# constantinpape/torch-em

Measured on AMD Instinct MI355X. Metric: voxels/sec fwd+bwd, UNet3d 1x128^3 bs=2, higher is better.
Workload: dtype f32-class (forward convs on normalised activations: fp32 operands split into 2 fp16 terms = 22 mantissa bits, lo plane scaled by 2^12 with its own fp32 accumulator, 3 fp16 MFMAs per product; other forward convs 3 bf16 terms / 6 MFMAs; data-gradient convs 2 bf16 terms / 3 MFMAs (16-bit products); WEI

## Files before the change

### torch_em_amd/csrc/conv1x1_stream.hip

```cpp
#include "tem_common.h"
#include "tem_act.h"
#include "conv_split.h"
#include "conv_internal.h"
#include "conv_arith.h"

template <int NS, bool F16, int CT, typename T>
__global__ __launch_bounds__(256) void k_conv1x1_stream(const T* __restrict__ x, int64_t x_ld,
                                                        const unsigned short* __restrict__ wp,
                                                        const float* __restrict__ bias, T* __restrict__ y,
                                                        int64_t y_ld, const T* __restrict__ ref, int64_t ref_ld,
                                                        int64_t NV, int Cin, int Cout, int act, int64_t nmt,
                                                        unsigned* __restrict__ amax) {
    const int lane = threadIdx.x & 63, wv = threadIdx.x >> 6;
    float amx = 0.f;
    const int r = lane & 31, kh = lane >> 5;
    const int ctg = blockIdx.y;
    const int nks = Cin >> 4;
    const uint4* wfrag = reinterpret_cast<const uint4*>(wp) + lane;
    for (int64_t mt = (int64_t)blockIdx.x * 4 + wv; mt < nmt; mt += (int64_t)gridDim.x * 4) {
        const int64_t v = mt * 32 + r;
        const bool vok = v < NV;
        const T* xr = x + (vok ? v : 0) * x_ld + kh * 8;
        floatx16 acc[CT];
#pragma unroll
        for (int ct = 0; ct < CT; ++ct)
#pragma unroll
            for (int k = 0; k < 16; ++k) acc[ct][k] = 0.f;
        for (int ks = 0; ks < nks; ++ks) {
            uint4 t[NS];
            if constexpr (sizeof(T) == 2) {
                static_assert(sizeof(T) == 4 || NS == 1, "16-bit storage: one-term modes only");
                t[0] = make_uint4(0u, 0u, 0u, 0u);
                if (vok) t[0] = *reinterpret_cast<const uint4*>(xr + ks * 16);
            } else {
                float4 a0 = make_float4(0.f, 0.f, 0.f, 0.f), a1 = a0;
                if (vok) {
                    a0 = act_ld4(xr + ks * 16);
                    a1 = act_ld4(xr + ks * 16 + 4);
                }
                float rem[8] = {a0.x, a0.y, a0.z, a0.w, a1.x, a1.y, a1.z, a1.w};
#pragma unroll
                for (int p = 0; p < NS; ++p) {
                    unsigned wds[4];
#pragma unroll
                    for (int e = 0; e < 4; ++e) {
                        const unsigned h = pk16<F16>(rem[2 * e], rem[2 * e + 1]);
                        wds[e] = h;
                        if (p + 1 < NS) {
                            rem[2 * e] -= lo16<F16>(h);
                            rem[2 * e + 1] -= hi16<F16>(h);
                        }
                    }
                    t[p] = make_uint4(wds[0], wds[1], wds[2], wds[3]);
                }
            }
#pragma unroll
            for (int ct = 0; ct < CT; ++ct) {
                const int nt = ctg * CT + ct;
                if (nt * 32 < Cout) {
                    const uint4* f = wfrag + ((int64_t)(nt * nks + ks) * NS) * 64;
                    uint4 b[NS];
#pragma unroll
                    for (int p = 0; p < NS; ++p) b[p] = f[p * 64];
#pragma unroll
                    for (int o = NS - 1; o >= 0; --o)
#pragma unroll
                        for (int i = 0; i <= o; ++i) acc[ct] = mfma16<F16>(b[o - i], t[i], acc[ct]);
                }
            }
        }
        if (vok) {
#pragma unroll
            for (int ct = 0; ct < CT; ++ct) {
#pragma unroll
                for (int q4 = 0; q4 < 4; ++q4) {
                    const int co = (ctg * CT + ct) * 32 + 8 * q4 + 4 * kh;
                    if (co < Cout) {
                        float4 o = make_float4(acc[ct][4 * q4], acc[ct][4 * q4 + 1], acc[ct][4 * q4 + 2], acc[ct][4 * q4 + 3]);
                        if (bias) {
                            const float4 b4 = *reinterpret_cast<const float4*>(bias + co);
                            o.x += b4.x;
                            o.y += b4.y;
                            o.z += b4.z;
                            o.w += b4.w;
                        }
                        o.x = act_apply_b(o.x, act);
                        o.y = act_apply_b(o.y, act);
                        o.z = act_apply_b(o.z, act);
                        o.w = act_apply_b(o.w, act);
                        if (ref) {
                            const float4 rv = act_ld4(ref + v * ref_ld + co);
                            o.x = rv.x > 0.f ? o.x : 0.f;
                            o.y = rv.y > 0.f ? o.y : 0.f;
                            o.z = rv.z > 0.f ? o.z : 0.f;
                            o.w = rv.w > 0.f ? o.w : 0.f;
                        }
                        act_st4(y + v * y_ld + co, o);
                        amx = tem_amax4(amx, o.x, o.y, o.z, o.w);
                    }
                }
            }
        }
    }
    if (amax) tem_amax_commit(amax, amx);
}

template <int NS, bool F16, typename T>
static void stream_launch(const TemConvCall& c, const T* x, int64_t x_ld, const float* wp, const float* bias, T* y, int64_t y_ld,
                          const T* ref, int64_t ref_ld, int64_t NV, int Cin, int Cout, int act, hipStream_t s) {
    const int64_t nmt = (NV + 31) / 32;
    const int ntile = Cout / 32;
    const int CT = ntile >= 2 ? 2 : 1;
    const int ngroups = (ntile + CT - 1) / CT;
    int64_t gx = (nmt + 3) / 4;
    if (gx > 8192) gx = 8192;
    const dim3 grid((unsigned)gx, (unsigned)ngroups);
    unsigned* const amax = c.take_output_amax();
    if (CT == 2)
        hipLaunchKernelGGL((k_conv1x1_stream<NS, F16, 2, T>), grid, dim3(256), 0, s, x, x_ld, (const unsigned short*)wp, bias, y, y_ld,
                           ref, ref_ld, NV, Cin, Cout, act, nmt, amax);
    else
        hipLaunchKernelGGL((k_conv1x1_stream<NS, F16, 1, T>), grid, dim3(256), 0, s, x, x_ld, (const unsigned short*)wp, bias, y, y_ld,
                           ref, ref_ld, NV, Cin, Cout, act, nmt, amax);
}

void tem_conv1x1_stream(const TemConvCall& c, const float* x, int64_t x_ld, const float* wp, const float* bias, float* y, int64_t y_ld,
                        const float* ref, int64_t ref_ld, const TemConvShape& sh, int act, int mode, hipStream_t s) {
    const int st = c.stx, Cin = sh.Cin, Cout = sh.Cout;
    const int64_t NV = sh.NV();
    auto go = [&](auto ns, auto f16, auto t) {
        using T = decltype(t);
        stream_launch<ns(), f16(), T>(c, (const T*)x, x_ld, wp, bias, (T*)y, y_ld, (const T*)ref, ref_ld, NV, Cin, Cout, act, s);
    };
    const TemArith& a = tem_arith(mode);
    if (st == TEM_ST_F16) go(TemInt<1>{}, TemBool<true>{}, tem_f16{});
    else if (st == TEM_ST_BF16) go(TemInt<1>{}, TemBool<false>{}, tem_bf16{});
    else if (a.planes == 3) go(TemInt<3>{}, TemBool<false>{}, float{});
    else if (a.planes == 2) go(TemInt<2>{}, TemBool<false>{}, float{});
    else tem_select_bool(a.elem == TEM_EL_F16, [&](auto f16) { go(TemInt<1>{}, f16, float{}); });
}
```

### torch_em_amd/csrc/capi.hip

```cpp
#include "tem_common.h"
#include "conv_internal.h"
#include "tem_act.h"
#include <stdarg.h>
#include <string.h>

static thread_local char g_err[512] = "";

void tem_set_error(const char* fmt, ...) {
    va_list ap;
    va_start(ap, fmt);
    vsnprintf(g_err, sizeof(g_err), fmt, ap);
    va_end(ap);
}

extern "C" const char* tem_last_error(void) { return g_err; }

struct TemOption {
    const char* name;
    long long def;
};
static const TemOption g_opt_table[TEM_OPT_COUNT] = {
    {"wgrad_zs", 3},
    {"wgrad_zs_persist", 1},
    {"wgrad_sums", 1},
    {"wgrad_sums_min_mb", 128},
    {"fwd_persistent", -1},
    {"conv_fwd_variant", -1},
    {"conv1x1_stream", 1},
    {"fwd_ksplit_chunks", 0},
    {"wgrad_cus", 256},
    {"upsample_generic", 0},
    {"team_min_units", 0},
    {"zr_splitk", 1},
    {"zr_wide", 1},
    {"zr_tile_blocks", 1},
    {"dice_vox", 1},
    {"upsample2_ch8", 1},
    {"pool_vec8", 2},
    {"fp32_zr", 1},
    {"zr_pair", 1},
};
static long long g_opt_val[TEM_OPT_COUNT];
static bool g_opt_set[TEM_OPT_COUNT];

long long tem_option(int id) {
    if (id < 0 || id >= TEM_OPT_COUNT) return 0;
    return __atomic_load_n(&g_opt_set[id], __ATOMIC_RELAXED) ? __atomic_load_n(&g_opt_val[id], __ATOMIC_RELAXED)
                                                            : g_opt_table[id].def;
}
static int opt_find(const char* name) {
    if (!name) return -1;
    for (int i = 0; i < TEM_OPT_COUNT; ++i)
        if (!strcmp(name, g_opt_table[i].name)) return i;
    return -1;
}
extern "C" int tem_set_option(const char* name, int64_t value) {
    const int id = opt_find(name);
    TEM_REQUIRE(id >= 0, "tem_set_option: unknown option '%s'", name ? name : "(null)");
    __atomic_store_n(&g_opt_val[id], (long long)value, __ATOMIC_RELAXED);
    __atomic_store_n(&g_opt_set[id], true, __ATOMIC_RELAXED);
    return TEM_OK;
}
extern "C" int tem_get_option(const char* name, int64_t* value) {
    const int id = opt_find(name);
    TEM_REQUIRE(id >= 0 && value, "tem_get_option: unknown option '%s'", name ? name : "(null)");
    *value = (int64_t)tem_option(id);
    return TEM_OK;
}
extern "C" int tem_version(void) { return 100; }

extern "C" int tem_device_cus(void) {
    int dev = 0;
    if (hipGetDevice(&dev) != hipSuccess) return TEM_ELAUNCH;
    hipDeviceProp_t prop;
    if (hipGetDeviceProperties(&prop, dev) != hipSuccess) return TEM_ELAUNCH;
    return prop.multiProcessorCount;
}
int tem_ncu() {
    static int ncu = 0;
    if (!ncu) {
        ncu = tem_device_cus();
        if (ncu <= 0) ncu = 256;
    }
    return ncu;
}

#define TT_V 64
#define TT_C 32

__global__ __launch_bounds__(256) void k_nchw_to_nhwc(const float* __restrict__ src, float* __restrict__ dst,
                                                      int64_t dst_ld, int C, int64_t V, int64_t vtiles, int ctiles) {
    __shared__ float tile[TT_C][TT_V + 1];
    int64_t ntiles = vtiles * ctiles;
    int n = blockIdx.y;
    for (int64_t t = blockIdx.x; t < ntiles; t += gridDim.x) {
        int ct = (int)(t % ctiles);
        int64_t vt = t / ctiles;
        int64_t v0 = vt * TT_V;
        int c0 = ct * TT_C;
        for (int i = threadIdx.x; i < TT_C * TT_V; i += 256) {
            int c = i / TT_V, v = i % TT_V;
            float val = 0.f;
            if (c0 + c < C && v0 + v < V) val = src[((int64_t)n * C + c0 + c) * V + v0 + v];
            tile[c][v] = val;
        }
        __syncthreads();
        for (int i = threadIdx.x; i < TT_C * TT_V; i += 256) {
            int v = i / TT_C, c = i % TT_C;
            if (c0 + c < C && v0 + v < V) dst[((int64_t)n * V + v0 + v) * dst_ld + c0 + c] = tile[c][v];
        }
        __syncthreads();
    }
}

__global__ __launch_bounds__(256) void k_nhwc_to_nchw(const float* __restrict__ src, int64_t src_ld,
                                                      float* __restrict__ dst, int C, int64_t V, int64_t vtiles,
                                                      int ctiles) {
    __shared__ float tile[TT_C][TT_V + 1];
    int64_t ntiles = vtiles * ctiles;
    int n = blockIdx.y;
    for (int64_t t = blockIdx.x; t < ntiles; t += gridDim.x) {
        int ct = (int)(t % ctiles);
        int64_t vt = t / ctiles;
        int64_t v0 = vt * TT_V;
        int c0 = ct * TT_C;
        for (int i = threadIdx.x; i < TT_C * TT_V; i += 256) {
            int v = i / TT_C, c = i % TT_C;
            float val = 0.f;
            if (c0 + c < C && v0 + v < V) val = src[((int64_t)n * V + v0 + v) * src_ld + c0 + c];
            tile[c][v] = val;
        }
        __syncthreads();
        for (int i = threadIdx.x; i < TT_C * TT_V; i += 256) {
            int c = i / TT_V, v = i % TT_V;
            if (c0 + c < C && v0 + v < V) dst[((int64_t)n * C + c0 + c) * V + v0 + v] = tile[c][v];
        }
        __syncthreads();
    }
}

extern "C" int tem_nchw_to_nhwc(const float* src, float* dst, int64_t dst_ld, int N, int C, int64_t V,
                                tem_stream_t stream) {
    TEM_REQUIRE(src && dst && N > 0 && C > 0 && V > 0 && dst_ld >= C, "tem_nchw_to_nhwc: bad arguments");
    int64_t vtiles = tem_cdiv(V, TT_V);
    int ctiles = (int)tem_cdiv(C, TT_C);
    int64_t nt = vtiles * ctiles;
    dim3 grid((unsigned)(nt > 4096 ? 4096 : nt), N);
    hipLaunchKernelGGL(k_nchw_to_nhwc, grid, dim3(256), 0, (hipStream_t)stream, src, dst, dst_ld, C, V, vtiles, ctiles);
    TEM_CHECK_LAUNCH("tem_nchw_to_nhwc");
    return TEM_OK;
}

extern "C" int tem_nhwc_to_nchw(const float* src, int64_t src_ld, float* dst, int N, int C, int64_t V,
                                tem_stream_t stream) {
    TEM_REQUIRE(src && dst && N > 0 && C > 0 && V > 0 && src_ld >= C, "tem_nhwc_to_nchw: bad arguments");
    int64_t vtiles = tem_cdiv(V, TT_V);
    int ctiles = (int)tem_cdiv(C, TT_C);
    int64_t nt = vtiles * ctiles;
    dim3 grid((unsigned)(nt > 4096 ? 4096 : nt), N);
    hipLaunchKernelGGL(k_nhwc_to_nchw, grid, dim3(256), 0, (hipStream_t)stream, src, src_ld, dst, C, V, vtiles, ctiles);
    TEM_CHECK_LAUNCH("tem_nhwc_to_nchw");
    return TEM_OK;
}

#define STD_BLOCKS 256

__global__ __launch_bounds__(256) void k_std_partial(const float* __restrict__ x, int64_t L, double* __restrict__ part) {
    int n = blockIdx.y;
    const float* row = x + (int64_t)n * L;
    double s = 0.0, ss = 0.0;
    for (int64_t i = (int64_t)blockIdx.x * 256 + threadIdx.x; i < L; i += (int64_t)gridDim.x * 256) {
        double v = (double)row[i];
        s += v;
        ss += v * v;
    }
    s = tem_wave_sum_d(s);
    ss = tem_wave_sum_d(ss);
    __shared__ double sh[2][4];
    int w = threadIdx.x >> 6;
    if ((threadIdx.x & 63) == 0) { sh[0][w] = s; sh[1][w] = ss; }
    __syncthreads();
    if (threadIdx.x == 0) {
        part[((int64_t)n * gridDim.x + blockIdx.x) * 2 + 0] = sh[0][0] + sh[0][1] + sh[0][2] + sh[0][3];
        part[((int64_t)n * gridDim.x + blockIdx.x) * 2 + 1] = sh[1][0] + sh[1][1] + sh[1][2] + sh[1][3];
    }
}

__global__ __launch_bounds__(256) void k_std_apply(const float* __restrict__ x, float* __restrict__ y, int64_t L,
                                                   const double* __restrict__ part, int nblk, float eps) {
    int n = blockIdx.y;
    __shared__ float sh_mean, sh_inv;
    if (threadIdx.x == 0) {
        double s = 0.0, ss = 0.0;
        for (int b = 0; b < nblk; ++b) {
            s += part[((int64_t)n * nblk + b) * 2 + 0];
            ss += part[((int64_t)n * nblk + b) * 2 + 1];
        }
        double mean = s / (double)L;
        double var = ss / (double)L - mean * mean;
        if (var < 0.0) var = 0.0;
        sh_mean = (float)mean;
        sh_inv = (float)(1.0 / (sqrt(var) + (double)eps));
    }
    __syncthreads();
    float mean = sh_mean, inv = sh_inv;
    const float* row = x + (int64_t)n * L;
    float* out = y + (int64_t)n * L;
    for (int64_t i = (int64_t)blockIdx.x * 256 + threadIdx.x; i < L; i += (int64_t)gridDim.x * 256)
        out[i] = (row[i] - mean) * inv;
}

extern "C" int tem_standardize(const float* x, float* y, int N, int64_t L, float eps, void* ws, int64_t ws_bytes,
                               tem_stream_t stream) {
    TEM_REQUIRE(x && y && ws && N > 0 && L > 0, "tem_standardize: bad arguments");
    int nblk = (int)(tem_cdiv(L, 256) < STD_BLOCKS ? tem_cdiv(L, 256) : STD_BLOCKS);
    if ((int64_t)N * nblk * 2 * (int64_t)sizeof(double) > ws_bytes) {
        tem_set_error("tem_standardize: workspace too small (%lld bytes needed)",
                      (long long)((int64_t)N * nblk * 2 * sizeof(double)));
        return TEM_EWS;
    }
    hipLaunchKernelGGL(k_std_partial, dim3(nblk, N), dim3(256), 0, (hipStream_t)stream, x, L, (double*)ws);
    hipLaunchKernelGGL(k_std_apply, dim3(nblk, N), dim3(256), 0, (hipStream_t)stream, x, y, L, (const double*)ws, nblk, eps);
    TEM_CHECK_LAUNCH("tem_standardize");
    return TEM_OK;
}

__global__ __launch_bounds__(256) void k_act_bwd(const float* __restrict__ gy, const float* __restrict__ y,
                                                 float* __restrict__ gx, int64_t n, int act) {
    for (int64_t i = (int64_t)blockIdx.x * 256 + threadIdx.x; i < n; i += (int64_t)gridDim.x * 256) {
        float yv = y[i], g = gy[i];
        gx[i] = (act == TEM_ACT_SIGMOID) ? g * yv * (1.f - yv) : ((yv > 0.f) ? g : 0.f);
    }
}

extern "C" int tem_act_bwd(const float* gy, const float* y, float* gx, int64_t n, int act, tem_stream_t stream) {
    TEM_REQUIRE(gy && y && gx && n > 0, "tem_act_bwd: bad arguments");
    TEM_REQUIRE(act == TEM_ACT_RELU || act == TEM_ACT_SIGMOID, "tem_act_bwd: Invalid activation: %d", act);
    hipLaunchKernelGGL(k_act_bwd, dim3(tem_grid_1d(n, 256)), dim3(256), 0, (hipStream_t)stream, gy, y, gx, n, act);
    TEM_CHECK_LAUNCH("tem_act_bwd");
    return TEM_OK;
}
```

### torch_em_amd/csrc/tem_common.h

```cpp
#pragma once
#include <hip/hip_runtime.h>
#include <stdint.h>
#include <stdio.h>
#include "../../include/tem_hip.h"

void tem_set_error(const char* fmt, ...);

enum {
    TEM_OPT_WGRAD_ZS = 0,
    TEM_OPT_WGRAD_ZS_PERSIST,
    TEM_OPT_WGRAD_SUMS,
    TEM_OPT_WGRAD_SUMS_MIN_MB,
    TEM_OPT_FWD_PERSISTENT,
    TEM_OPT_CONV_FWD_VARIANT,
    TEM_OPT_CONV1X1_STREAM,
    TEM_OPT_FWD_KSPLIT_CHUNKS,
    TEM_OPT_WGRAD_CUS,
    TEM_OPT_UPSAMPLE_GENERIC,
    TEM_OPT_TEAM_MIN_UNITS,
    TEM_OPT_ZR_SPLITK,
    TEM_OPT_ZR_WIDE,
    TEM_OPT_ZR_TILE_BLOCKS,
    TEM_OPT_DICE_VOX,
    TEM_OPT_UPSAMPLE2_CH8,
    TEM_OPT_POOL_VEC8,
    TEM_OPT_FP32_ZR,
    TEM_OPT_ZR_PAIR,
    TEM_OPT_COUNT
};
long long tem_option(int id);
int tem_ncu();

#define TEM_REQUIRE(cond, ...)                 \
    do {                                       \
        if (!(cond)) {                         \
            tem_set_error(__VA_ARGS__);        \
            return TEM_EINVAL;                 \
        }                                      \
    } while (0)

#define TEM_TRY(call)                          \
    do {                                       \
        const int rc__ = (call);               \
        if (rc__ != TEM_OK) return rc__;       \
    } while (0)

#define TEM_CHECK_LAUNCH(name)                                                   \
    do {                                                                         \
        hipError_t e__ = hipGetLastError();                                      \
        if (e__ != hipSuccess) {                                                 \
            tem_set_error("%s: launch failed: %s", name, hipGetErrorString(e__)); \
            return TEM_ELAUNCH;                                                  \
        }                                                                        \
    } while (0)

static inline int64_t tem_cdiv(int64_t a, int64_t b) { return (a + b - 1) / b; }
static inline int64_t tem_align_up(int64_t a, int64_t b) { return tem_cdiv(a, b) * b; }

static inline int tem_grid_1d(int64_t work_items, int block, int max_blocks = 256 * 8) {
    int64_t g = tem_cdiv(work_items, block);
    if (g > max_blocks) g = max_blocks;
    if (g < 1) g = 1;
    return (int)g;
}

#define TEM_WAVE 64

__device__ __forceinline__ float tem_amax4(float m, float a, float b, float c, float d) {
    return __builtin_fmaxf(__builtin_fmaxf(m, __builtin_fmaxf(__builtin_fabsf(a), __builtin_fabsf(b))),
                           __builtin_fmaxf(__builtin_fabsf(c), __builtin_fabsf(d)));
}
__device__ __forceinline__ void tem_amax_commit(unsigned* amax, float m) {
    unsigned u = __builtin_bit_cast(unsigned, m);
#pragma unroll
    for (int o = 32; o > 0; o >>= 1) u = max(u, (unsigned)__shfl_xor((int)u, o, 64));
    if ((threadIdx.x & 63) == 0 && u > __atomic_load_n(amax, __ATOMIC_RELAXED)) atomicMax(amax, u);
}

__device__ __forceinline__ float tem_wave_sum(float v) {
#pragma unroll
    for (int o = 32; o > 0; o >>= 1) v += __shfl_xor(v, o, 64);
    return v;
}
__device__ __forceinline__ double tem_wave_sum_d(double v) {
#pragma unroll
    for (int o = 32; o > 0; o >>= 1) v += __shfl_xor(v, o, 64);
    return v;
}

__device__ __forceinline__ int tem_xcd_remap(int bid, int nwg) {
    const int nx = 8;
    int q = nwg / nx, r = nwg % nx;
    int xcd = bid % nx, idx = bid / nx;
    int base = (xcd < r) ? xcd * (q + 1) : r * (q + 1) + (xcd - r) * q;
    return base + idx;
}
```

Before: 281.8 million.

## Stage 1x1 conv stream I/O through per-wave LDS with coalesced loads and prefetch

Rewrites the 1x1 streaming conv so each wave loads input rows with coalesced 16-byte requests into a per-wave LDS slab and reads MFMA fragments from there. The next channel chunk and the next tile are prefetched into registers while the current one computes. Outputs are transposed through LDS so the epilogue issues row-contiguous stores and ref-mask loads. The grid becomes persistent, sized from CU count and a waves-per-EU hint, and the old per-lane kernel stays available behind an option. This targets strided global access in the old kernel, at the cost of LDS use, extra wave barriers and changed occupancy, and the CT choice now differs when Cout exceeds 64.

Result: no change. 283.3 million, median of 6 (+0.5%).

```diff
diff --git a/torch_em_amd/csrc/conv1x1_stream.hip b/torch_em_amd/csrc/conv1x1_stream.hip
--- a/torch_em_amd/csrc/conv1x1_stream.hip
+++ b/torch_em_amd/csrc/conv1x1_stream.hip
@@ -4,8 +4,203 @@
 #include "conv_internal.h"
 #include "conv_arith.h"
 
+#define S1_ROWB 144
+#define S1_WAVE_LDS(CT) (32 * (128 * (CT) + 16))
+#ifndef TEM_S1_WG_PER_CU
+#define TEM_S1_WG_PER_CU 0
+#endif
+
+__device__ __forceinline__ void s1_wave_lds_order() {
+    __builtin_amdgcn_fence(__ATOMIC_RELEASE, "wavefront");
+    __builtin_amdgcn_wave_barrier();
+    __builtin_amdgcn_fence(__ATOMIC_ACQUIRE, "wavefront");
+}
+
+template <int NS, bool F16>
+__device__ __forceinline__ void s1_split(const float4 a0, const float4 a1, uint4 (&t)[NS]) {
+    float rem[8] = {a0.x, a0.y, a0.z, a0.w, a1.x, a1.y, a1.z, a1.w};
+#pragma unroll
+    for (int p = 0; p < NS; ++p) {
+        unsigned wds[4];
+#pragma unroll
+        for (int e = 0; e < 4; ++e) {
+            const unsigned h = pk16<F16>(rem[2 * e], rem[2 * e + 1]);
+            wds[e] = h;
+            if (p + 1 < NS) {
+                rem[2 * e] -= lo16<F16>(h);
+                rem[2 * e + 1] -= hi16<F16>(h);
+            }
+        }
+        t[p] = make_uint4(wds[0], wds[1], wds[2], wds[3]);
+    }
+}
+
+template <int CT, bool MASK, typename T>
+__device__ __forceinline__ float s1_store_rows(char* lb, const floatx16 (&acc)[CT], const float* __restrict__ bias, T* __restrict__ y,
+                                               int64_t y_ld, const T* __restrict__ ref, int64_t ref_ld, int64_t v0, int64_t NV, int co0,
+                                               int act, int lane, float amx) {
+    constexpr int LPV = 8 * CT, VPI = 64 / LPV, NK = 32 / VPI, ROWB = 128 * CT + 16;
+    static_assert(32 * ROWB <= S1_WAVE_LDS(CT), "slab");
+    const int r = lane & 31, kh = lane >> 5;
+    const int row = lane / LPV, c4 = lane % LPV;
+    const int co = co0 + c4 * 4;
+    const int nv = NV - v0 < 32 ? (int)(NV - v0) : 32;
+    float4 b4 = make_float4(0.f, 0.f, 0.f, 0.f);
+    if (bias) b4 = *reinterpret_cast<const float4*>(bias + co);
+    const T* const rp = ref + (v0 + row) * ref_ld + co;
+    const T* const rlast = ref + (v0 + nv - 1) * ref_ld + co;
+    T* const yp = y + (v0 + row) * y_ld + co;
+    auto ref_rows = [&](int k0, float4 (&rv)[4]) {
+#pragma unroll
+        for (int k = 0; k < 4; ++k)
+            if constexpr (MASK) rv[k] = act_ld4(row + (k0 + k) * VPI < nv ? rp + (k0 + k) * VPI * ref_ld : rlast);
+    };
+    float4 rv[4], rvn[4];
+    ref_rows(0, rv);
+    s1_wave_lds_order();
+#pragma unroll
+    for (int ct = 0; ct < CT; ++ct)
+#pragma unroll
+        for (int q4 = 0; q4 < 4; ++q4)
+            *reinterpret_cast<float4*>(lb + r * ROWB + (ct * 32 + 8 * q4 + 4 * kh) * 4) =
+                make_float4(acc[ct][4 * q4], acc[ct][4 * q4 + 1], acc[ct][4 * q4 + 2], acc[ct][4 * q4 + 3]);
+    s1_wave_lds_order();
+#pragma unroll
+    for (int k0 = 0; k0 < NK; k0 += 4) {
+        float4 o[4];
+#pragma unroll
+        for (int k = 0; k < 4; ++k) o[k] = *reinterpret_cast<const float4*>(lb + ((k0 + k) * VPI + row) * ROWB + c4 * 16);
+#pragma unroll
+        for (int k = 0; k < 4; ++k) {
+            if (bias) {
+                o[k].x += b4.x;
+                o[k].y += b4.y;
+                o[k].z += b4.z;
+                o[k].w += b4.w;
+            }
+            o[k].x = act_apply_b(o[k].x, act);
+            o[k].y = act_apply_b(o[k].y, act);
+            o[k].z = act_apply_b(o[k].z, act);
+            o[k].w = act_apply_b(o[k].w, act);
+            if constexpr (MASK) {
+                o[k].x = rv[k].x > 0.f ? o[k].x : 0.f;
+                o[k].y = rv[k].y > 0.f ? o[k].y : 0.f;
+                o[k].z = rv[k].z > 0.f ? o[k].z : 0.f;
+                o[k].w = rv[k].w > 0.f ? o[k].w : 0.f;
+            }
+        }
+        __builtin_amdgcn_sched_barrier(0);
+        if (k0 + 4 < NK) ref_rows(k0 + 4, rvn);
+#pragma unroll
+        for (int k = 0; k < 4; ++k)
+            if (row + (k0 + k) * VPI < nv) {
+                act_st4(yp + (k0 + k) * VPI * y_ld, o[k]);
+                amx = tem_amax4(amx, o[k].x, o[k].y, o[k].z, o[k].w);
+            }
+        __builtin_amdgcn_sched_barrier(0);
+#pragma unroll
+        for (int k = 0; k < 4; ++k) rv[k] = rvn[k];
+    }
+    return amx;
+}
+
+#ifndef TEM_S1_WAVES2
+#define TEM_S1_WAVES2 4
+#endif
+#define S1_WAVES(CT) ((CT) == 2 ? TEM_S1_WAVES2 : 5)
+template <int NS, bool F16, int CT, bool MASK, typename T>
+__global__ __launch_bounds__(256) __attribute__((amdgpu_waves_per_eu(S1_WAVES(CT))))
+void k_conv1x1_stream(const T* __restrict__ x, int64_t x_ld,
+                                                        const unsigned short* __restrict__ wp,
+                                                        const float* __restrict__ bias, T* __restrict__ y,
+                                                        int64_t y_ld, const T* __restrict__ ref, int64_t ref_ld,
+                                                        int64_t NV, int Cin, int Cout, int act, int64_t nmt,
+                                                        unsigned* __restrict__ amax) {
+    static_assert(sizeof(T) == 4 || NS == 1, "16-bit storage: one-term modes only");
+    constexpr int EPP = 16 / sizeof(T);
+    constexpr int KSC = EPP / 2;
+    __shared__ uint4 slab[4 * S1_WAVE_LDS(CT) / 16];
+    const int lane = threadIdx.x & 63;
+    const int wv = __builtin_amdgcn_readfirstlane(threadIdx.x >> 6);
+    char* const lb = reinterpret_cast<char*>(slab) + wv * S1_WAVE_LDS(CT);
+    float amx = 0.f;
+    const int r = lane & 31, kh = lane >> 5;
+    const int pc = lane & 7, vq = lane >> 3;
+    const int ctg = blockIdx.y;
+    const int nks = Cin >> 4;
+    const int nch = (nks + KSC - 1) / KSC;
+    const uint4* wfrag = reinterpret_cast<const uint4*>(wp) + lane;
+    const int64_t mstep = (int64_t)gridDim.x * 4;
+    int64_t mt = (int64_t)blockIdx.x * 4 + wv;
+    uint4 ld[4];
+    auto request = [&](int64_t m, int c) {
+        const int e = (c * 8 + pc) * EPP;
+#pragma unroll
+        for (int j = 0; j < 4; ++j) {
+            const int64_t v = m * 32 + j * 8 + vq;
+            ld[j] = make_uint4(0u, 0u, 0u, 0u);
+            if (v < NV && e < Cin) ld[j] = *reinterpret_cast<const uint4*>(x + v * x_ld + e);
+        }
+    };
+    if (mt < nmt) request(mt, 0);
+    while (mt < nmt) {
+        floatx16 acc[CT];
+#pragma unroll
+        for (int ct = 0; ct < CT; ++ct)
+#pragma unroll
+            for (int k = 0; k < 16; ++k) acc[ct][k] = 0.f;
+        for (int c = 0; c < nch; ++c) {
+            s1_wave_lds_order();
+#pragma unroll
+            for (int j = 0; j < 4; ++j) *reinterpret_cast<uint4*>(lb + (j * 8 + vq) * S1_ROWB + pc * 16) = ld[j];
+            s1_wave_lds_order();
+            if (c + 1 < nch) request(mt, c + 1);
+#pragma unroll 1
+            for (int ksl = 0; ksl < KSC; ++ksl) {
+                const int ks = c * KSC + ksl;
+                if (ks < nks) {
+                    uint4 t[NS];
+                    if constexpr (sizeof(T) == 2) {
+                        t[0] = *reinterpret_cast<const uint4*>(lb + r * S1_ROWB + ksl * 32 + kh * 16);
+                    } else {
+                        const char* p = lb + r * S1_ROWB + ksl * 64 + kh * 32;
+                        s1_split<NS, F16>(*reinterpret_cast<const float4*>(p), *reinterpret_cast<const float4*>(p + 16), t);
+                    }
+                    constexpr int GB = CT * NS <= 3 ? CT : 1;
+#pragma unroll
+                    for (int c0 = 0; c0 < CT; c0 += GB) {
+                        uint4 b[GB][NS];
+#pragma unroll
+                        for (int ct = c0; ct < c0 + GB; ++ct) {
+                            const int nt = ctg * CT + ct;
+                            if (nt * 32 < Cout) {
+                                const uint4* f = wfrag + ((int64_t)(nt * nks + ks) * NS) * 64;
+#pragma unroll
+                                for (int p = 0; p < NS; ++p) b[ct - c0][p] = f[p * 64];
+                            }
+                        }
+#pragma unroll
+                        for (int ct = c0; ct < c0 + GB; ++ct) {
+                            if ((ctg * CT + ct) * 32 < Cout) {
+#pragma unroll
+                                for (int o = NS - 1; o >= 0; --o)
+#pragma unroll
+                                    for (int i = 0; i <= o; ++i) acc[ct] = mfma16<F16>(b[ct - c0][o - i], t[i], acc[ct]);
+                            }
+                        }
+                    }
+                }
+            }
+        }
+        if (mt + mstep < nmt) request(mt + mstep, 0);
+        amx = s1_store_rows<CT, MASK>(lb, acc, bias, y, y_ld, ref, ref_ld, mt * 32, NV, ctg * CT * 32, act, lane, amx);
+        mt += mstep;
+    }
+    if (amax) tem_amax_commit(amax, amx);
+}
+
 template <int NS, bool F16, int CT, typename T>
-__global__ __launch_bounds__(256) void k_conv1x1_stream(const T* __restrict__ x, int64_t x_ld,
+__global__ __launch_bounds__(256) void k_conv1x1_stream_lane(const T* __restrict__ x, int64_t x_ld,
                                                         const unsigned short* __restrict__ wp,
                                                         const float* __restrict__ bias, T* __restrict__ y,
                                                         int64_t y_ld, const T* __restrict__ ref, int64_t ref_ld,
@@ -110,18 +305,28 @@
                           const T* ref, int64_t ref_ld, int64_t NV, int Cin, int Cout, int act, hipStream_t s) {
     const int64_t nmt = (NV + 31) / 32;
     const int ntile = Cout / 32;
-    const int CT = ntile >= 2 ? 2 : 1;
+    const bool lane_io = tem_option(TEM_OPT_CONV1X1_STREAM) == 2;
+    const int CT = ntile == 2 || (lane_io && ntile > 2) ? 2 : 1;
     const int ngroups = (ntile + CT - 1) / CT;
     int64_t gx = (nmt + 3) / 4;
-    if (gx > 8192) gx = 8192;
+    int64_t gmax = lane_io ? 8192 : (int64_t)tem_ncu() * (TEM_S1_WG_PER_CU ? TEM_S1_WG_PER_CU : S1_WAVES(CT)) / ngroups;
+    if (gmax < 1) gmax = 1;
+    if (gx > gmax) gx = gmax;
     const dim3 grid((unsigned)gx, (unsigned)ngroups);
     unsigned* const amax = c.take_output_amax();
-    if (CT == 2)
-        hipLaunchKernelGGL((k_conv1x1_stream<NS, F16, 2, T>), grid, dim3(256), 0, s, x, x_ld, (const unsigned short*)wp, bias, y, y_ld,
-                           ref, ref_ld, NV, Cin, Cout, act, nmt, amax);
-    else
-        hipLaunchKernelGGL((k_conv1x1_stream<NS, F16, 1, T>), grid, dim3(256), 0, s, x, x_ld, (const unsigned short*)wp, bias, y, y_ld,
-                           ref, ref_ld, NV, Cin, Cout, act, nmt, amax);
+    auto go = [&](auto kern) {
+        hipLaunchKernelGGL(kern, grid, dim3(256), 0, s, x, x_ld, (const unsigned short*)wp, bias, y, y_ld, ref, ref_ld, NV, Cin, Cout, act,
+                           nmt, amax);
+    };
+    if (lane_io) {
+        if (CT == 2) go(k_conv1x1_stream_lane<NS, F16, 2, T>);
+        else go(k_conv1x1_stream_lane<NS, F16, 1, T>);
+    } else {
+        tem_select_bool(ref != nullptr, [&](auto mask) {
+            if (CT == 2) go(k_conv1x1_stream<NS, F16, 2, mask(), T>);
+            else go(k_conv1x1_stream<NS, F16, 1, mask(), T>);
+        });
+    }
 }
 
 void tem_conv1x1_stream(const TemConvCall& c, const float* x, int64_t x_ld, const float* wp, const float* bias, float* y, int64_t y_ld,
```

## Stage 1x1 conv activations through swizzled LDS for coalesced row loads and stores

Applied to the files above, without the earlier changes.

Adds a new fp32 1x1-conv streaming kernel, on by default through a new option. Each wave loads 32-voxel tiles as full contiguous channel lines, transposes them into a per-wave swizzled LDS slab, and prefetches the next 32-channel chunk while the MFMAs run. Epilogue results also go through LDS so stores are coalesced row lines instead of strided per-lane float4 writes. It costs extra LDS traffic, wave barriers, and more register pressure under tightened launch bounds. The epilogue only handles ReLU or no activation, not the general act_apply_b path.

New measurement: 281.7 million before, 282.4 million after (median of 6 runs). About the same (+0.3%).

```diff
diff --git a/torch_em_amd/csrc/capi.hip b/torch_em_amd/csrc/capi.hip
--- a/torch_em_amd/csrc/capi.hip
+++ b/torch_em_amd/csrc/capi.hip
@@ -39,6 +39,7 @@
     {"pool_vec8", 2},
     {"fp32_zr", 1},
     {"zr_pair", 1},
+    {"c1x1_lines", 1},
 };
 static long long g_opt_val[TEM_OPT_COUNT];
 static bool g_opt_set[TEM_OPT_COUNT];
diff --git a/torch_em_amd/csrc/conv1x1_stream.hip b/torch_em_amd/csrc/conv1x1_stream.hip
--- a/torch_em_amd/csrc/conv1x1_stream.hip
+++ b/torch_em_amd/csrc/conv1x1_stream.hip
@@ -105,6 +105,171 @@
     if (amax) tem_amax_commit(amax, amx);
 }
 
+#define C1L_SLAB 256
+typedef float c1l_f4 __attribute__((ext_vector_type(4)));
+__device__ __forceinline__ void c1l_lds_written() { asm volatile("s_waitcnt lgkmcnt(0)" ::: "memory"); }
+template <int NS, bool F16, int CT>
+__global__ __launch_bounds__(256, (NS == 3 && CT == 2) ? 3 : 4) void k_conv1x1_stream_lines(const float* __restrict__ x, int64_t x_ld,
+                                                              const unsigned short* __restrict__ wp,
+                                                              const float* __restrict__ bias, float* __restrict__ y,
+                                                              int64_t y_ld, const float* __restrict__ ref, int64_t ref_ld,
+                                                              int64_t NV, int Cin, int Cout, int act, int64_t nmt,
+                                                              unsigned* __restrict__ amax) {
+    __shared__ c1l_f4 lds[4 * C1L_SLAB];
+    const int lane = threadIdx.x & 63, wv = __builtin_amdgcn_readfirstlane(threadIdx.x >> 6);
+    float amx = 0.f;
+    const int r = lane & 31, kh = lane >> 5;
+    const int lr = lane >> 3, lp = lane & 7;
+    c1l_f4* const slab = lds + wv * C1L_SLAB;
+    c1l_f4* const vrow = slab + r * 8;
+    const int swz_in = (r >> 1) & 7, swz_out = r & 7;
+    const int ctg = blockIdx.y;
+    const int nks = Cin >> 4, nkp = (nks + 1) >> 1;
+    const bool relu = act == TEM_ACT_RELU;
+    const uint4* wfrag = reinterpret_cast<const uint4*>(wp) + lane;
+    const unsigned xo = ((unsigned)lr * (unsigned)x_ld + lp * 4) * 4u, x8 = 32u * (unsigned)x_ld;
+    const unsigned yo = ((unsigned)lr * (unsigned)y_ld + lp * 4) * 4u, y8 = 32u * (unsigned)y_ld;
+    const unsigned ro = ((unsigned)lr * (unsigned)ref_ld + lp * 4) * 4u, r8 = 32u * (unsigned)ref_ld;
+    for (int64_t mt = (int64_t)blockIdx.x * 4 + wv; mt < nmt; mt += (int64_t)gridDim.x * 4) {
+        const int64_t left = NV - mt * 32;
+        const int rows = left < 32 ? (int)left : 32;
+        const char* const xt = reinterpret_cast<const char*>(x + mt * 32 * x_ld);
+        const char* const rt = reinterpret_cast<const char*>(ref + mt * 32 * ref_ld);
+        char* const yt = reinterpret_cast<char*>(y + mt * 32 * y_ld);
+        unsigned xoff[4], roff[4];
+#pragma unroll
+        for (int j = 0; j < 4; ++j) {
+            const bool live = 8 * j + lr < rows;
+            xoff[j] = live ? xo + j * x8 : 0u;
+            roff[j] = live ? ro + j * r8 + (unsigned)(ctg * CT * 128) : 0u;
+        }
+        floatx16 acc[CT];
+#pragma unroll
+        for (int ct = 0; ct < CT; ++ct)
+#pragma unroll
+            for (int k = 0; k < 16; ++k) acc[ct][k] = 0.f;
+        c1l_f4 cur[4];
+#pragma unroll
+        for (int j = 0; j < 4; ++j) cur[j] = *reinterpret_cast<const c1l_f4*>(xt + (lp * 4 < Cin ? xoff[j] : 0u));
+        for (int kp = 0; kp < nkp; ++kp) {
+#pragma unroll
+            for (int j = 0; j < 4; ++j) {
+                const int row = 8 * j + lr;
+                slab[row * 8 + (lp ^ ((row >> 1) & 7))] = cur[j];
+            }
+            c1l_lds_written();
+            if (kp + 1 < nkp) {
+                const bool pok = (kp + 1) * 32 + lp * 4 < Cin;
+#pragma unroll
+                for (int j = 0; j < 4; ++j) cur[j] = *reinterpret_cast<const c1l_f4*>(xt + (pok ? xoff[j] + (unsigned)((kp + 1) * 128) : 0u));
+            }
+#pragma unroll
+            for (int s = 0; s < 2; ++s) {
+                const int ks = 2 * kp + s;
+                if (ks < nks) {
+                    const c1l_f4 u0 = vrow[(4 * s + 2 * kh) ^ swz_in], u1 = vrow[(4 * s + 2 * kh + 1) ^ swz_in];
+                    float rem[8] = {u0.x, u0.y, u0.z, u0.w, u1.x, u1.y, u1.z, u1.w};
+                    uint4 t[NS];
+#pragma unroll
+                    for (int p = 0; p < NS; ++p) {
+                        unsigned wds[4];
+#pragma unroll
+                        for (int e = 0; e < 4; ++e) {
+                            const unsigned h = pk16<F16>(rem[2 * e], rem[2 * e + 1]);
+                            wds[e] = h;
+                            if (p + 1 < NS) {
+                                rem[2 * e] -= lo16<F16>(h);
+                                rem[2 * e + 1] -= hi16<F16>(h);
+                            }
+                        }
+                        t[p] = make_uint4(wds[0], wds[1], wds[2], wds[3]);
+                    }
+#pragma unroll
+                    for (int ct = 0; ct < CT; ++ct) {
+                        const int nt = ctg * CT + ct;
+                        if (nt * 32 < Cout) {
+                            const uint4* f = wfrag + ((int64_t)(nt * nks + ks) * NS) * 64;
+                            uint4 b[NS];
+#pragma unroll
+                            for (int p = 0; p < NS; ++p) b[p] = f[p * 64];
+#pragma unroll
+                            for (int o = NS - 1; o >= 0; --o)
+#pragma unroll
+                                for (int i = 0; i <= o; ++i) acc[ct] = mfma16<F16>(b[o - i], t[i], acc[ct]);
+                        }
+                    }
+                }
+            }
+            __builtin_amdgcn_wave_barrier();
+        }
+        c1l_f4 rv[CT][4];
+#pragma unroll
+        for (int ct = 0; ct < CT; ++ct)
+#pragma unroll
+            for (int j = 0; j < 4; ++j) rv[ct][j] = c1l_f4{0.f, 0.f, 0.f, 0.f};
+        if (ref) {
+#pragma unroll
+            for (int j = 0; j < 4; ++j) rv[0][j] = *reinterpret_cast<const c1l_f4*>(rt + roff[j]);
+        }
+#pragma unroll
+        for (int ct = 0; ct < CT; ++ct) {
+            const int nt = ctg * CT + ct;
+            if (nt * 32 < Cout) {
+                float4 b4[4];
+#pragma unroll
+                for (int q4 = 0; q4 < 4; ++q4) b4[q4] = make_float4(0.f, 0.f, 0.f, 0.f);
+                if (bias) {
+#pragma unroll
+                    for (int q4 = 0; q4 < 4; ++q4) b4[q4] = *reinterpret_cast<const float4*>(bias + nt * 32 + 8 * q4 + 4 * kh);
+                }
+#pragma unroll
+                for (int q4 = 0; q4 < 4; ++q4) {
+                    float4 o = make_float4(acc[ct][4 * q4], acc[ct][4 * q4 + 1], acc[ct][4 * q4 + 2], acc[ct][4 * q4 + 3]);
+                    if (bias) {
+                        o.x += b4[q4].x;
+                        o.y += b4[q4].y;
+                        o.z += b4[q4].z;
+                        o.w += b4[q4].w;
+                    }
+                    o.x = (relu & !(o.x > 0.f)) ? 0.f : o.x;
+                    o.y = (relu & !(o.y > 0.f)) ? 0.f : o.y;
+                    o.z = (relu & !(o.z > 0.f)) ? 0.f : o.z;
+                    o.w = (relu & !(o.w > 0.f)) ? 0.f : o.w;
+                    vrow[(2 * q4 + kh) ^ swz_out] = c1l_f4{o.x, o.y, o.z, o.w};
+                }
+                c1l_lds_written();
+                if (ct + 1 < CT && ref && (nt + 1) * 32 < Cout) {
+#pragma unroll
+                    for (int j = 0; j < 4; ++j)
+                        rv[ct + 1 < CT ? ct + 1 : ct][j] = *reinterpret_cast<const c1l_f4*>(rt + (roff[j] + (unsigned)((ct + 1) * 128)));
+                }
+                auto store_tile = [&](auto full) {
+#pragma unroll
+                    for (int j = 0; j < 4; ++j) {
+                        const int row = 8 * j + lr;
+                        const c1l_f4 u = slab[row * 8 + (lp ^ (row & 7))];
+                        float4 o = make_float4(u.x, u.y, u.z, u.w);
+                        if (ref) {
+                            o.x = rv[ct][j].x > 0.f ? o.x : 0.f;
+                            o.y = rv[ct][j].y > 0.f ? o.y : 0.f;
+                            o.z = rv[ct][j].z > 0.f ? o.z : 0.f;
+                            o.w = rv[ct][j].w > 0.f ? o.w : 0.f;
+                        }
+                        if (full() || row < rows) {
+                            act_st4(reinterpret_cast<float*>(yt + (yo + j * y8 + (unsigned)(nt * 128))), o);
+                            amx = tem_amax4(amx, o.x, o.y, o.z, o.w);
+                        }
+                    }
+                };
+                if (rows == 32) store_tile(TemBool<true>{});
+                else store_tile(TemBool<false>{});
+                __builtin_amdgcn_wave_barrier();
+            }
+        }
+    }
+    if (amax) tem_amax_commit(amax, amx);
+}
+
 template <int NS, bool F16, typename T>
 static void stream_launch(const TemConvCall& c, const T* x, int64_t x_ld, const float* wp, const float* bias, T* y, int64_t y_ld,
                           const T* ref, int64_t ref_ld, int64_t NV, int Cin, int Cout, int act, hipStream_t s) {
@@ -116,6 +281,17 @@
     if (gx > 8192) gx = 8192;
     const dim3 grid((unsigned)gx, (unsigned)ngroups);
     unsigned* const amax = c.take_output_amax();
+    if constexpr (sizeof(T) == 4) {
+        if (tem_option(TEM_OPT_C1X1_LINES)) {
+            if (CT == 2)
+                hipLaunchKernelGGL((k_conv1x1_stream_lines<NS, F16, 2>), grid, dim3(256), 0, s, x, x_ld, (const unsigned short*)wp, bias, y,
+                                   y_ld, ref, ref_ld, NV, Cin, Cout, act, nmt, amax);
+            else
+                hipLaunchKernelGGL((k_conv1x1_stream_lines<NS, F16, 1>), grid, dim3(256), 0, s, x, x_ld, (const unsigned short*)wp, bias, y,
+                                   y_ld, ref, ref_ld, NV, Cin, Cout, act, nmt, amax);
+            return;
+        }
+    }
     if (CT == 2)
         hipLaunchKernelGGL((k_conv1x1_stream<NS, F16, 2, T>), grid, dim3(256), 0, s, x, x_ld, (const unsigned short*)wp, bias, y, y_ld,
                            ref, ref_ld, NV, Cin, Cout, act, nmt, amax);
diff --git a/torch_em_amd/csrc/tem_common.h b/torch_em_amd/csrc/tem_common.h
--- a/torch_em_amd/csrc/tem_common.h
+++ b/torch_em_amd/csrc/tem_common.h
@@ -26,6 +26,7 @@
     TEM_OPT_POOL_VEC8,
     TEM_OPT_FP32_ZR,
     TEM_OPT_ZR_PAIR,
+    TEM_OPT_C1X1_LINES,
     TEM_OPT_COUNT
 };
 long long tem_option(int id);
```
